# NUStatBioinfo/DegNorm

Measured on AMD Instinct MI355X. Metric: genes/sec (20k genes x 10 samples, 5 iters), higher is better.
Workload: dtype f64

## Files before the change

### degnorm_amd/csrc/dn_api.hip

```cpp
#include "dn_kernels.hpp"
#include "dn_host.hpp"
#include "dn_outer.hpp"
#include "../../include/degnorm_amd.h"

#include <dlfcn.h>
#include <rccl/rccl.h>

#include <algorithm>
#include <atomic>
#include <cmath>
#include <cstdio>
#include <cstdlib>
#include <cstring>
#include <memory>
#include <numeric>
#include <string>
#include <thread>
#include <vector>

#ifndef DN_P_MAX_TEMPLATED
#define DN_P_MAX_TEMPLATED 64
#endif
#define DN_P_2_16(X)  X(2) X(3) X(4) X(5) X(6) X(7) X(8) X(9) X(10) X(11) X(12) X(13) X(14) X(15) X(16)
#define DN_P_17_24(X) X(17) X(18) X(19) X(20) X(21) X(22) X(23) X(24)
// ... 299 lines not shown
#ifndef DN_BUILD_STAMP
#define DN_BUILD_STAMP "unknown build"
#endif
const char *dn_version(void) { return "degnorm_amd 0.2.0 (gfx950) [" DN_BUILD_STAMP "]"; }
const char *dn_last_error(void) { return dn::last_error(); }
const char *dn_reads_last_error(void) { return dn::last_error(); }
const char *dn_assemble_last_error(void) { return dn::last_error(); }
const char *dn_gtf_last_error(void) { return dn::last_error(); }

int dn_device_count(void)
{
    int n = 0;
    if (hipGetDeviceCount(&n) != hipSuccess) return 0;
    return n;
}

int dn_p_supported(int p) { return p <= dn::P_MAX && dn::kernel_set_for(p) != nullptr; }
int dn_p_max(void) { return dn::P_WIDE_MAX; }

static int create_streams(dn_handle h)
{
    int prio_least = 0, prio_greatest = 0;
    DN_TRY(hipDeviceGetStreamPriorityRange(&prio_least, &prio_greatest));
    const int prio[dn_handle_s::NCLS] = {prio_greatest, (prio_least + prio_greatest) / 2, prio_least};
    for (int c = 0; c < dn_handle_s::NCLS; c++) {
        DN_TRY(h->stream[c].create(hipStreamCreateWithPriority, hipStreamNonBlocking, prio[c]));
        DN_TRY(h->ev_start[c].create(hipEventCreate));
        DN_TRY(h->ev_end[c].create(hipEventCreate));
        DN_TRY(h->ev_mid[c].create(hipEventCreateWithFlags, hipEventDisableTiming));
    }
    DN_TRY(h->ev_ready.create(hipEventCreateWithFlags, hipEventDisableTiming));
    DN_TRY(h->ev_i0.create(hipEventCreate));
    DN_TRY(h->ev_i1.create(hipEventCreate));
    return DN_OK;
}

int dn_create(int device, dn_handle *out)
{
    if (!out) return fail(DN_E_INVALID, "dn_create: out is null");
    *out = nullptr;
    int ndev = 0;
    if (hipGetDeviceCount(&ndev) != hipSuccess || ndev <= 0) return fail(DN_E_NO_DEVICE, "no HIP device visible");
    if (device < 0 || device >= ndev) return fail(DN_E_INVALID, "dn_create: device index out of range");
    DN_TRY(hipSetDevice(device));
    hipDeviceProp_t prop;
    DN_TRY(hipGetDeviceProperties(&prop, device));
    dn_handle h = std::make_unique<dn_handle_s>().release();
    h->device = device;
    h->n_cus = prop.multiProcessorCount;
    const int rc = create_streams(h);
    if (rc != DN_OK) {
        const std::string msg = g_err;
        (void) dn_destroy(h);
        return fail(rc, msg);
    }
    *out = h;
    return DN_OK;
}

int dn_destroy(dn_handle h)
{
    if (!h) return DN_OK;
    (void) hipSetDevice(h->device);
    wait_streams(h);
    (void) dn_comm_destroy(h);
    delete h;
    return DN_OK;
}

static int64_t lds_tier_cols(const dn::KernelSet *ks, int per_cu, int32_t p)
{
    const int64_t lds_per_block = (160 * 1024) / per_cu - (int64_t) ks->static_lds_bytes - 256;
    const int64_t ps = p + (p & 1);
    return lds_per_block > 0 ? lds_per_block / std::max(1, ks->units) / (8 * ps) : 0;
}

static int size_class(dn_handle h, dn_handle_s::GeneClass &C, int32_t cols)
{
    const int32_t p = h->p;
    int per_cu = C.ks->blocks_per_cu(0);
    if (per_cu < 1) per_cu = 1;
    const int units = std::max(1, C.ks->units);
    int slots = (int) std::min<int64_t>(((int64_t) C.n + units - 1) / units * units, (int64_t) per_cu * h->n_cus * units);
    const int32_t S = (cols + 63) & ~63;
    const int64_t slot_bytes = (int64_t) S * ((int64_t) p * 2 * sizeof(float) + (int64_t) (p + (p & 1)) * sizeof(double) + 3 * sizeof(double)) +
                               (int64_t) C.ks->slot_extra_bytes;
    {
        size_t free_b = 0, total_b = 0;
        DN_TRY(hipMemGetInfo(&free_b, &total_b));
        const int64_t budget = (int64_t) ((free_b + (C.d_ws ? (size_t) C.slot_bytes * (size_t) std::max(C.slots, 1) : 0)) / 3);
        if (slot_bytes > budget) return fail(DN_E_INVALID, "a gene is too long for the device scratch (" + std::to_string(S) + " columns)");
        slots = (int) std::max<int64_t>(units, std::min<int64_t>(slots, budget / slot_bytes / units * units));
    }
    dn::DeviceBuffer<char> ws;
    DN_TRY(ws.alloc((size_t) slot_bytes * (size_t) std::max(slots, 1)));
    C.d_ws = std::move(ws);
    C.slots = slots; C.S = S; C.slot_bytes = slot_bytes;
    const int64_t lcols = std::min<int64_t>(lds_tier_cols(C.ks, per_cu, p), C.S) & ~(int64_t) 1;
    C.lds_cols = (int32_t) lcols;
    C.dyn_lds = (size_t) units * (size_t) lcols * 8 * (size_t) (p + (p & 1));
    return DN_OK;
}

struct CoverageSource {
    const float *packed = nullptr;
    const void *const *genes = nullptr;
    int32_t is_f32 = 0, n_threads = 1;
    std::atomic<int64_t> *bad = nullptr;
};

static void pack_genes(dn_handle h, const CoverageSource &src, int64_t g0, int64_t g1, float *stage)
{
    const int32_t p = h->p;
    const int64_t base = h->goff[g0];
    std::atomic<int64_t> next(g0);
    auto work = [&]() {
        int64_t local_bad = 0;
        for (;;) {
            const int64_t a = next.fetch_add(16);
            if (a >= g1) break;
            const int64_t b = std::min(g1, a + 16);
            for (int64_t g = a; g < b; g++) {
                const int64_t cnt = (int64_t) p * h->glen[g];
                float *dst = stage + (h->goff[g] - base);
                if (src.is_f32) std::memcpy(dst, src.genes[g], sizeof(float) * (size_t) cnt);
                else {
                    const double *s = (const double *) src.genes[g];
                    for (int64_t k = 0; k < cnt; k++) { const float f = (float) s[k]; dst[k] = f; local_bad += ((double) f != s[k]); }
                }
            }
        }
        if (src.bad) *src.bad += local_bad;
    };
    const int nt = (int) std::max<int64_t>(1, std::min<int64_t>(src.n_threads, (g1 - g0 + 15) / 16));
    std::vector<std::thread> th;
    for (int t = 1; t < nt; t++) th.emplace_back(work);
    work();
    for (auto &t : th) t.join();
}

static int upload_ragged_chunks(dn_handle h, const CoverageSource &src, dn::PinnedBuffer<float> (&stage)[2], dn::Event (&done)[2])
{
    const int64_t n = h->n;
    int64_t chunk = (int64_t) 32 << 20;
    if (const char *env = getenv("DN_UPLOAD_CHUNK_FLOATS")) chunk = std::max<int64_t>(1, atoll(env));
    for (int64_t g = 0; g < n; g++) chunk = std::max(chunk, (int64_t) h->p * h->glen[g]);
    chunk = std::min(chunk, std::max<int64_t>(h->total, 1));
    for (int b = 0; b < 2; b++) {
        if (stage[b].alloc(sizeof(float) * (size_t) chunk) != hipSuccess ||
            done[b].create(hipEventCreateWithFlags, hipEventDisableTiming) != hipSuccess) return fail(DN_E_HIP, "upload: pinned staging buffer");
    }
    int64_t g0 = 0;
    for (int k = 0; g0 < n; k++) {
        int64_t g1 = g0, fl = 0;
        while (g1 < n && fl + (int64_t) h->p * h->glen[g1] <= chunk) { fl += (int64_t) h->p * h->glen[g1]; g1++; }
        const int b = k & 1;
        if (k >= 2 && hipEventSynchronize(done[b]) != hipSuccess) return fail(DN_E_HIP, "upload: event");
        pack_genes(h, src, g0, g1, stage[b]);
        if (hipMemcpyAsync(h->data.d_cov + h->goff[g0], stage[b], sizeof(float) * (size_t) fl, hipMemcpyHostToDevice, h->stream[0]) != hipSuccess ||
            hipEventRecord(done[b], h->stream[0]) != hipSuccess) return fail(DN_E_HIP, "upload: copy");
        g0 = g1;
    }
    if (hipStreamSynchronize(h->stream[0]) != hipSuccess) return fail(DN_E_HIP, "upload: synchronize");
    return DN_OK;
}

static void class_lengths(const dn::KernelSet *ks, int32_t p, int32_t &split_len, int32_t &tiny_len, const dn::KernelSet *&pair)
{
    {
        const char *env = getenv("DN_SPLIT_LEN");
        const dn::KernelSet *narrow = (ks->p != 0) ? dn::kernel_set_narrow(p) : nullptr;
        split_len = 0;
        if (env) split_len = atoi(env);
        else if (narrow) {
            const int64_t lds_cols_n = lds_tier_cols(narrow, std::max(1, narrow->blocks_per_cu(0)), p);
            const int64_t reg_cols_n = narrow->reg_tier_cols;
            split_len = (int32_t) (reg_cols_n > 0 ? (int64_t) (1.775 * (double) (reg_cols_n + lds_cols_n)) : (int64_t) (2.1 * (double) lds_cols_n));
        }
        if (!narrow) split_len = 0;
        if (!env && p >= 25) split_len = 0;
        pair = (ks->p != 0 && split_len > 0) ? dn::kernel_set_pair(p) : nullptr;
// ... 1072 lines not shown
```

### degnorm_amd/csrc/dn_kernels.hpp

```cpp
#pragma once
#include <hip/hip_runtime.h>
#include <stddef.h>
#include <stdint.h>
#include <type_traits>
#include "dn_reduce.hpp"
#include "dn_dpp_ops.hpp"

#ifdef DN_MARKS
#define DN_MARK(name) asm volatile("; DN_MARK " name)
#else
#define DN_MARK(name)
#endif

namespace dn {

constexpr int TRACE_LEN = 48;
constexpr int MAX_BINS = 64;
constexpr int P_MAX = 64;
constexpr int P_WIDE_MAX = 256;

enum { EXIT_LOW_COV = 0, EXIT_ZERO_SAMPLE = 1, EXIT_MEDIAN = 2, EXIT_NO_LOOP = 3,
       EXIT_REFINED = 4, EXIT_REFINE_FALLBACK = 5, EXIT_NOT_FOUND_FALLBACK = 6 };
enum { LOOP_NATURAL = 0, LOOP_PERFECT = 1, LOOP_VALUE_ERROR = 2, LOOP_ZERO_ROWSUM = 3, LOOP_MIN_BINS = 4,
       LOOP_NOT_ENTERED = 5 };
enum { ST_OK = 0, ST_ARPACK = -1, ST_EMPTY_MIN = -2, ST_VALUE_ERROR = -3,
       ST_NO_CONVERGENCE = -4 };
constexpr int EIG_MAX_STEPS_DEFAULT = 4000;
enum { EM_INPUT = 0,
       EM_EXPAND = 1,
       EM_REFINED = 2,
       EM_CLAMPED = 3,
       EM_RAW = 4 };

template <typename CovT>
struct IterFields {
    const CovT    *cov;
    const int64_t *goff;
    const int32_t *glen;
    const int32_t *order;
    int32_t       *counter;
    const int64_t *ds_start;
    const CovT    *rowmax;
    const int32_t *x16;
    char          *ws;
    double        *rho;
    int32_t       *flags;
    int32_t       *trace;
    double        *kfin;
    int32_t       *emode;
    double        *svec;
    const int64_t *svoff;
    int64_t        slot_bytes;
    int32_t        n_genes;
    int32_t        S;
    int32_t        lds_cols;
    int32_t        T, bins, min_hc, rate, skip, want_est;
    int32_t        p;
    int32_t        max_steps;
    int32_t        handdown_cols;
    int32_t       *hand_int;
    double        *hand_dbl;
    int32_t       *park_queue;
    int32_t       *park_count;
    const int32_t *resume_queue;
    const int32_t *resume_count;
};
constexpr int HAND_MAX_BINS = 32;
constexpr int HAND_INTS = 16 + HAND_MAX_BINS;

struct IterArgs : IterFields<float> { double scale[P_MAX], inv_scale[P_MAX]; };

struct IterArgsF64 : IterFields<double> { double scale[P_MAX], inv_scale[P_MAX]; };

struct WideIterArgs : IterFields<float> { const double *scale, *inv_scale; };

struct InitArgs {
    const float   *cov;
    const int64_t *goff;
    const int32_t *glen;
    const int32_t *order;
    int32_t       *counter;
    double        *est_sums;
    double        *cov_sums;
    int32_t       *status;
    int32_t        n_genes;
    int32_t        p;
    int32_t        max_steps;
    char          *ws;
    int64_t        slot_bytes;
    int32_t        S;
    const int32_t *x16;
    int32_t        force_fp64;
};

template <typename CovT>
struct EstFields {
    const CovT    *cov;
    const int64_t *goff;
    const int32_t *glen;
    const double  *kfin;
    const int32_t *emode;
    const double  *svec;
    const int64_t *svoff;
    double        *out;
    const int64_t *ooff;
    int32_t        n_genes;
    int32_t        p;
};
struct EstArgs : EstFields<float> { double scale[P_MAX]; };
struct EstArgsF64 : EstFields<double> { double scale[P_MAX]; };
struct WideEstArgs : EstFields<float> { const double *scale; };

#pragma clang diagnostic push
#pragma clang diagnostic ignored "-Winvalid-offsetof"
template <typename A> constexpr bool iter_layout_kept()
{
    return sizeof(A) == 1256 && offsetof(A, slot_bytes) == 128 && offsetof(A, p) == 172 && offsetof(A, hand_int) == 184 &&
           offsetof(A, scale) == 232 && offsetof(A, inv_scale) == 744;
}
template <typename A> constexpr bool est_layout_kept() { return sizeof(A) == 592 && offsetof(A, p) == 76 && offsetof(A, scale) == 80; }
static_assert(iter_layout_kept<IterArgs>() && iter_layout_kept<IterArgsF64>(), "IterArgs / IterArgsF64: layout moved");
static_assert(est_layout_kept<EstArgs>() && est_layout_kept<EstArgsF64>(), "EstArgs / EstArgsF64: layout moved");
#pragma clang diagnostic pop

struct NmfArgsF64 {
    const double  *x;
    const int64_t *xoff;
    const int32_t *ncol;
    const int64_t *eoff;
    const int32_t *order;
    int32_t       *counter;
    double        *K;
    double        *E;
    double        *est;
    int32_t       *status;
    char          *ws;
    int64_t        slot_bytes;
    int32_t        n, p, T, ratio, max_steps;
};

#ifndef DN_MG_MIN_P
#define DN_MG_MIN_P 25
#endif

template <int P, int NT>
struct Smem {
    static constexpr int W = NT / 64;
    static constexpr int MG_TR = (P + 15) / 16;
    static constexpr int MG_STR = 16 * MG_TR;
// ... 768 lines not shown
#define g_sm g_sm_u[DN_UNIT]
#define g_gs g_gs_u[DN_UNIT]
typedef const float __attribute__((address_space(1))) *gF_cptr;
typedef double __attribute__((address_space(1))) *gdouble_ptr;

template <int P>
__device__ __forceinline__ void col_update(const double (&f)[P], double (&a)[P], const double (&u)[P], const double (&ur)[P], double c)
{
    double s0 = 0.0, s1 = 0.0;
#pragma unroll
    for (int i = 0; i + 1 < P; i += 2) { s0 = fma(u[i], a[i], s0); s1 = fma(u[i + 1], a[i + 1], s1); }
    if (P & 1) s0 = fma(u[P - 1], a[P - 1], s0);
    const double s = s0 + s1;
#pragma unroll
    for (int i = 0; i < P; i++) {
        const double res = fma(ur[i], s, -f[i]);
        a[i] = fmax(fma(-c, res, a[i]), f[i]);
    }
}

template <int P>
__device__ __forceinline__ void col_update_lds(const float (&x)[P], const double *invp, double (&a)[P], const double *uv, double c)
{
    double s0 = 0.0, s1 = 0.0;
#pragma unroll
    for (int i = 0; i + 1 < P; i += 2) {
        const double2 u2 = *reinterpret_cast<const double2 *>(uv + i);
        s0 = fma(u2.x, a[i], s0); s1 = fma(u2.y, a[i + 1], s1);
    }
    if (P & 1) s0 = fma(uv[P - 1], a[P - 1], s0);
    const double s = s0 + s1;
#pragma unroll
    for (int i = 0; i < P; i++) {
        const double fi = (double) x[i] * invp[i];
        const double res = fma(uv[i], s, -fi);
        a[i] = fmax(fma(-c, res, a[i]), fi);
    }
}

template <int P>
__device__ __forceinline__ void col_final(const double (&f)[P], const double (&a)[P], const double (&u)[P], bool first,
                                          double (&acc)[2 * P + 1], double &s_out, double &r_out)
{
    double s = 0.0;
#pragma unroll
    for (int i = 0; i < P; i++) s = fma(u[i], a[i], s);
    acc[0] += s;
    double rmax = 0.0;
#pragma unroll
    for (int i = 0; i < P; i++) {
        const double ke = u[i] * s;
        acc[1 + i] += ke < f[i] ? f[i] : ke;
        acc[1 + P + i] += f[i];
        double d = ke - f[i];
        if (!first) d = d < 0.0 ? 0.0 : d;
        const double r = d * rcp_newton(f[i] + 1.0);
        const double r2 = r * r;
        rmax = r2 > rmax ? r2 : rmax;
    }
    s_out = s; r_out = rmax;
}

template <int PS>
__device__ __forceinline__ void lds_col_read(const double *col, double (&a)[PS])
{
#pragma unroll
    for (int i = 0; i < PS; i += 2) { const double2 v = *reinterpret_cast<const double2 *>(col + i); a[i] = v.x; a[i + 1] = v.y; }
}
template <int PS>
__device__ __forceinline__ void lds_col_write(double *col, const double (&a)[PS])
{
#pragma unroll
    for (int i = 0; i < PS; i += 2) *reinterpret_cast<double2 *>(col + i) = make_double2(a[i], a[i + 1]);
}

typedef float dn_f4 __attribute__((ext_vector_type(4)));
typedef float dn_f2 __attribute__((ext_vector_type(2)));
typedef dn_f4 dn_f4u __attribute__((aligned(4)));
typedef dn_f2 dn_f2u __attribute__((aligned(4)));
typedef const dn_f4u __attribute__((address_space(1))) *gF4_cptr;
typedef const dn_f2u __attribute__((address_space(1))) *gF2_cptr;

template <int P>
__device__ __forceinline__ void load_x(gF_cptr Fb, int k, float (&x)[P])
{
    gF_cptr col = Fb + (size_t) k * P;
#pragma unroll
    for (int i = 0; i + 4 <= P; i += 4) {
        const dn_f4 v = *(gF4_cptr) (col + i);
        x[i] = v.x; x[i + 1] = v.y; x[i + 2] = v.z; x[i + 3] = v.w;
    }
    if constexpr ((P & 3) >= 2) {
        const dn_f2 v = *(gF2_cptr) (col + (P & ~3));
        x[P & ~3] = v.x; x[(P & ~3) + 1] = v.y;
    }
    if constexpr (P & 1) x[P - 1] = col[P - 1];
}

template <int P>
__device__ __forceinline__ void load_f(gF_cptr Fb, int k, const double (&inv)[P], double (&f)[P])
{
    float x[P];
    load_x<P>(Fb, k, x);
#pragma unroll
    for (int i = 0; i < P; i++) f[i] = (double) x[i] * inv[i];
}

template <int P, bool RAW>
__device__ __forceinline__ void pass_counts(const float (&x)[P], const double (&inv)[P], double (&f)[P])
{
#pragma unroll
    for (int i = 0; i < P; i++) f[i] = RAW ? (double) x[i] : (double) x[i] * inv[i];
}

typedef double dn_d2 __attribute__((ext_vector_type(2)));
typedef dn_d2 __attribute__((address_space(1))) *gd2_ptr;
template <int P> constexpr int spill_mid() { return (P + (P & 1)) / 4; }
template <int P>
__device__ __forceinline__ gd2_ptr spill_col(gdouble_ptr Lg, int k)
{
    constexpr int PS = P + (P & 1);
    gd2_ptr col = (gd2_ptr) (Lg + ((size_t) (k >> 6) * (64 * PS) + (size_t) (k & 63) * 2)) + spill_mid<P>() * 64;
    asm volatile("" : "+v"(col));
    return col;
}
template <int P>
__device__ __forceinline__ void spill_col_read(gd2_ptr col, double (&a)[P])
{
#pragma unroll
    for (int q = 0; q < (P + 1) / 2; q++) {
        const dn_d2 v = col[(q - spill_mid<P>()) * 64];
        a[2 * q] = v.x;
        if (2 * q + 1 < P) a[2 * q + 1] = v.y;
    }
}
template <int P>
__device__ __forceinline__ void spill_col_write(gd2_ptr col, const double (&a)[P])
{
#pragma unroll
    for (int q = 0; q < (P + 1) / 2; q++) col[(q - spill_mid<P>()) * 64] = dn_d2{a[2 * q], 2 * q + 1 < P ? a[2 * q + 1 < P ? 2 * q + 1 : 2 * q] : 0.0};
}

template <int P, int NT>
__device__ __forceinline__ int mg_core(gF_cptr Fb, gdouble_ptr Lg, double *lam, int n, int nL, int T,
                                       double (&u)[P], double &theta, int &steps, int maxs, bool &noconv)
{
    constexpr int W = NT / 64;
    constexpr int NG = P * (P + 1) / 2;
    constexpr int PS = P + (P & 1);
    constexpr int TR = Smem<P, NT>::MG_TR, STR = Smem<P, NT>::MG_STR;
    constexpr int NTILE = TR * (TR + 1) / 2;
    Smem<P, NT> &sm = g_sm;
    const int tid = DN_TIDX, lane = lane_id(), w = wave_id();
    const int nLe = (n < nL) ? n : nL;
    double *stage = &sm.stage[w * 16 * STR];
    double *uv = &sm.eigv[w * 128], *vv = uv + 64;
    const double *invp = g_gs.inv;
    for (int e = lane; e < 16 * STR; e += 64) stage[e] = 0.0;
    uv[lane] = lane < P ? 1.0 / sqrt((double) P) : 0.0;
    vv[lane] = 0.0;
    wave_fence();
    const int oi = lane & 15, okq = lane >> 4;
    dn_double4 acc[NTILE];

    auto feed = [&](const double (&a)[PS], bool valid) {
#pragma unroll
        for (int cq = 0; cq < 4; cq++) {
            if ((lane >> 4) == cq) {
                double *dst = stage + (lane & 15) * STR;
#pragma unroll
                for (int i = 0; i < PS; i += 2) *reinterpret_cast<double2 *>(dst + i) = make_double2(valid ? a[i] : 0.0, valid ? a[i + 1] : 0.0);
            }
            wave_fence();
#pragma unroll
            for (int g = 0; g < 4; g++) {
                double x[TR];
#pragma unroll
                for (int tr = 0; tr < TR; tr++) x[tr] = stage[(4 * g + okq) * STR + 16 * tr + oi];
                int tix = 0;
// ... 192 lines not shown
template <int IDX> __device__ __forceinline__ void agpr_put(double v)
{
    agpr_put1<IDX>(__double2loint(v));
    agpr_put1<IDX + 1>(__double2hiint(v));
}

template <int P, int BASE> __device__ __forceinline__ void rt_read(double (&a)[P])
{
    static_for<0, P>([&](auto ic) { constexpr int I = decltype(ic)::value; a[I] = agpr_get<BASE + 2 * I>(); });
}
template <int P, int BASE> __device__ __forceinline__ void rt_write(const double (&a)[P])
{
    static_for<0, P>([&](auto ic) { constexpr int I = decltype(ic)::value; agpr_put<BASE + 2 * I>(a[I]); });
}
template <int P, int BASE> __device__ __forceinline__ void rt_read_counts(double (&xd)[P])
{
    static_for<0, (P + 1) / 2>([&](auto jc) {
        constexpr int J = decltype(jc)::value;
        const unsigned w = (unsigned) agpr_get1<BASE + J>();
        xd[2 * J] = (double) (w & 0xffffu);
        if constexpr (2 * J + 1 < P) xd[2 * J + 1] = (double) (w >> 16);
    });
}
template <int P, int BASE> __device__ __forceinline__ void rt_write_counts(const float (&x)[P])
{
    static_for<0, (P + 1) / 2>([&](auto jc) {
        constexpr int J = decltype(jc)::value;
        unsigned w = (unsigned) x[2 * J];
        if constexpr (2 * J + 1 < P) w |= ((unsigned) x[2 * J + 1]) << 16;
        agpr_put1<BASE + J>((int) w);
    });
}
template <int P, bool X16> constexpr int rt_col_regs() { return 2 * P + (X16 ? (P + 1) / 2 : 0); }
template <int P, bool X16> constexpr int rt_cols()
{
    return (P >= DN_RT_MIN_P && P <= DN_RT_MAX_P) ? (256 / rt_col_regs<P, X16>() < DN_RT_MAX_COLS ? 256 / rt_col_regs<P, X16>() : DN_RT_MAX_COLS) : 0;
}
template <int P> constexpr int rt_regs_used()
{
    return rt_cols<P, true>() * rt_col_regs<P, true>() > rt_cols<P, false>() * rt_col_regs<P, false>()
               ? rt_cols<P, true>() * rt_col_regs<P, true>() : rt_cols<P, false>() * rt_col_regs<P, false>();
}
constexpr int RT_BATCH = 48;
#define DN_RT_SAVE_IDX(r) ((size_t) (r) * NT + DN_TIDX)
template <int N, int NT> __device__ __forceinline__ void rt_save(int *save, int need)
{
    static_for<0, (N + RT_BATCH - 1) / RT_BATCH>([&](auto bc) {
        constexpr int B = decltype(bc)::value * RT_BATCH;
        constexpr int CNT = (N - B) < RT_BATCH ? (N - B) : RT_BATCH;
        if (B < need) {
            int v[CNT];
            static_for<0, CNT>([&](auto ic) { constexpr int I = decltype(ic)::value; v[I] = agpr_get1<B + I>(); });
#pragma unroll
            for (int i = 0; i < CNT; i++) save[DN_RT_SAVE_IDX(B + i)] = v[i];
            asm volatile("" ::: "memory");
        }
    });
}
template <int N, int NT> __device__ __forceinline__ void rt_restore(const int *save, int need)
{
    static_for<0, (N + RT_BATCH - 1) / RT_BATCH>([&](auto bc) {
        constexpr int B = decltype(bc)::value * RT_BATCH;
        constexpr int CNT = (N - B) < RT_BATCH ? (N - B) : RT_BATCH;
        if (B < need) {
            int v[CNT];
#pragma unroll
            for (int i = 0; i < CNT; i++) v[i] = save[DN_RT_SAVE_IDX(B + i)];
            static_for<0, CNT>([&](auto ic) { constexpr int I = decltype(ic)::value; agpr_put1<B + I>(v[I]); });
            asm volatile("" ::: "memory");
        }
    });
}
template <int R, int RT, typename F>
__device__ __forceinline__ void partial_rounds(int nr, F &&column)
{
    if constexpr (R < RT) {
        if (R == 0 || R < nr) {
            column(std::integral_constant<int, R>{});
            __builtin_amdgcn_sched_barrier(0);
            partial_rounds<R + 1, RT>(nr, column);
        }
    }
}
template <int P, int NT> constexpr size_t rt_save_bytes() { return (size_t) rt_regs_used<P>() * 4 * NT; }

template <int P, int NT, bool X16, bool FULL = false, bool ONCHIP = false, bool SAFE = false>
__device__ __forceinline__ void nmf_body(const float *Fb_, double *Lg_, double *rs_, double *sv_,
                                         int n, int S, int nL, int T, int first_i)
{
    Smem<P, NT> &sm = g_sm;
    double *lam = g_lam + (DN_UNITS > 1 ? (size_t) DN_UNIT * (size_t) nL * (P + (P & 1)) : 0);
    gF_cptr Fb = (gF_cptr) uniform_ptr(Fb_);
    gdouble_ptr Lg = (gdouble_ptr) uniform_ptr(Lg_);
    gdouble_ptr rs = (gdouble_ptr) uniform_ptr(rs_);
    gdouble_ptr sv = (gdouble_ptr) uniform_ptr(sv_);
    n = __builtin_amdgcn_readfirstlane(n);
    S = __builtin_amdgcn_readfirstlane(S);
    nL = __builtin_amdgcn_readfirstlane(nL);
    T = __builtin_amdgcn_readfirstlane(T);
    const bool first = __builtin_amdgcn_readfirstlane(first_i) != 0;
    double inv[P], u[P], theta = 0.0;
    int steps = 0;
    const int maxs = __builtin_amdgcn_readfirstlane(g_gs.max_steps);
    bool noconv = false;
#pragma unroll
    for (int i = 0; i < P; i++) inv[i] = uniform(g_gs.inv[i]);
    long long stamp[4] = {0, 0, 0, 0};
#ifdef DN_STAMP
#define DN_T0() const long long t0_ = __builtin_amdgcn_s_memtime()
#define DN_T1(slot) stamp[slot] += __builtin_amdgcn_s_memtime() - t0_
#else
#define DN_T0()
#define DN_T1(slot) (void) stamp
#endif
    constexpr int NG = P * (P + 1) / 2;
    constexpr int CH_MAX = P <= 15 ? 120 : 90;
    constexpr int SW = (NG + CH_MAX - 1) / CH_MAX;
    constexpr int CH = (NG + SW - 1) / SW;
    constexpr int PS = P + (P & 1);
    const int tid = DN_TIDX;
    constexpr int RT = DN_REG_TIER ? rt_cols<P, X16>() : 0;
    constexpr int CS = rt_col_regs<P, X16>();
    constexpr int NR = RT * NT;
    constexpr bool RAW = raw_units<P>();
    double ud[P], ur[P];
    const int nLe = (n < NR + nL) ? n : NR + nL;
    const int kS0 = NR + nL;
    if constexpr (P >= DN_MG_MIN_P) {
        const int st = mg_core<P, NT>(Fb, Lg, lam, n, nL, T, u, theta, steps, maxs, noconv);
        if (st != ST_OK) { if (tid == 0) g_gs.status = st; dn_sync(); return; }
    } else {
    gram_t G[CH];

#ifdef DN_STAMP
    const long long t_cold0 = __builtin_amdgcn_s_memtime();
#endif
#pragma unroll
    for (int i = 0; i < CH; i++) G[i] = 0.0;
    {
        float xq[P];
        if (tid < n) load_x<P>(Fb, tid, xq);
#pragma clang loop unroll(disable)
        for (int k = tid; k < n; k += NT) {
            double f[P];
#pragma unroll
            for (int i = 0; i < P; i++) f[i] = (double) xq[i] * inv[i];
            load_x<P>(Fb, k + NT < n ? k + NT : k, xq);
            gram_add_range<P, 0, CH>(G, f);
        }
    }
    block_sum_lds<CH, P, NT, gram_t>(G, sm);
    static_for<1, SW>([&](auto qc) {
        constexpr int Q = decltype(qc)::value;
        constexpr int NQ = (NG - Q * CH) < CH ? (NG - Q * CH) : CH;
        gram_t Gq[NQ];
#pragma unroll
        for (int i = 0; i < NQ; i++) Gq[i] = 0.0;
#pragma clang loop unroll(disable)
        for (int k = tid; k < n; k += NT) {
            double f[P];
            load_f<P>(Fb, k, inv, f);
            gram_add_range<P, Q * CH, NQ>(Gq, f);
        }
        block_sum_lds<NQ, P, NT, gram_t, false, Q * CH>(Gq, g_sm);
    });
    {
        double tr = 0.0;
#pragma unroll
        for (int i = 0; i < P; i++) tr += sm.tot[i * (i + 1) / 2 + i];
        if (!(tr > 0.0)) { if (tid == 0) g_gs.status = ST_ARPACK; dn_sync(); return; }
    }
    Solver<P> solver;
    {
        double tr = 0.0;
#pragma unroll
        for (int i = 0; i < P; i++) tr += sm.tot[i * (i + 1) / 2 + i];
        solver.cold(tr, u);
    }
    {
        const int r = SAFE ? solve_by_blocks<P>(solver, sm.tot, Smem<P, NT>::ZSLOT, u, theta, maxs)
                           : solver.run(sm.tot, Smem<P, NT>::ZSLOT, u, theta, T == 0, maxs, true);
        steps += r; noconv = noconv || r > maxs;
    }
    const double c = 1.0 / sqrt((double) T);
    auto pass_u = [&]() {
        if constexpr (RAW) {
            const int k = Solver<P>::row_of_lane() < P ? Solver<P>::row_of_lane() : P - 1;
            const double vt = solver.iterate_of_row() * g_gs.inv[k], vh = solver.iterate_of_row() * g_gs.scl[k];
#pragma unroll
            for (int i = 0; i < P; i++) { ud[i] = Solver<P>::bcast_component(vt, i); ur[i] = Solver<P>::bcast_component(vh, i); }
        } else {
#pragma unroll
            for (int i = 0; i < P; i++) { u[i] = uniform(u[i]); ud[i] = u[i]; ur[i] = u[i]; }
        }
    };
    pass_u();

    constexpr bool PART = RT > 0 && X16 && !FULL;
    const int nr = (n + NT - 1) / NT;
    static_for<0, RT>([&](auto rc) {
        constexpr int R = decltype(rc)::value;
        const int k = tid + R * NT;
        if constexpr (PART) {
            if (R < nr) {
                float xf[P];
                double f[P];
#pragma unroll
                for (int i = 0; i < P; i++) xf[i] = 0.0f;
                if (k < n) load_x<P>(Fb, k, xf);
                pass_counts<P, RAW>(xf, inv, f);
                rt_write<P, CS * R>(f);
                rt_write_counts<P, CS * R + 2 * P>(xf);
            }
        } else if (k < n) {
            float xf[P];
            double f[P];
            load_x<P>(Fb, k, xf);
            pass_counts<P, RAW>(xf, inv, f);
            rt_write<P, CS * R>(f);
            if constexpr (X16) rt_write_counts<P, CS * R + 2 * P>(xf);
        }
    });
    for (int k = NR + tid; k < nLe; k += NT) {
        double f[P], a[PS];
        { float xf[P]; load_x<P>(Fb, k, xf); pass_counts<P, RAW>(xf, inv, f); }
#pragma unroll
        for (int i = 0; i < PS; i++) a[i] = i < P ? f[i] : 0.0;
        lds_col_write<PS>(lam + (size_t) (k - NR) * PS, a);
    }
    if constexpr (!ONCHIP) {
        for (int k = kS0 + tid; k < n; k += NT) {
            double f[P];
            { float xf[P]; load_x<P>(Fb, k, xf); pass_counts<P, RAW>(xf, inv, f); }
            spill_col_write<P>(spill_col<P>(Lg, k), f);
        }
    }
#ifdef DN_STAMP
    stamp[3] += __builtin_amdgcn_s_memtime() - t_cold0;
#endif
    constexpr bool G0 = FULL && ONCHIP && SW == 1;
    constexpr bool SQ = Solver<P>::SQUARE && SW == 1 && !SAFE;
#pragma clang loop unroll(disable)
    for (int t = 0; t < T; t++) {
        DN_MARK("iter_begin");
        auto gram_zero = [&]() {
#pragma unroll
            for (int i = 0; i < CH; i++) G[i] = 0.0;
        };
        if constexpr (!G0 && !PART) gram_zero();
        DN_MARK("zeroed");
        { DN_T0();
        const int dir = (t & 1) ? -1 : 1;

        auto reg_tier = [&](auto start) {
            if constexpr (RT > 0 && X16) {
                auto column = [&](auto rc) {
                    constexpr int R = decltype(rc)::value;
                    double f[P], a[P];
                    rt_read_counts<P, CS * R + 2 * P>(f);
                    if constexpr (!RAW) {
#pragma unroll
                        for (int i = 0; i < P; i++) f[i] *= inv[i];
                    }
                    rt_read<P, CS * R>(a);
                    col_update<P>(f, a, ud, ur, c);
                    if constexpr (decltype(start)::value && R == 0) gram_set_range<P, 0, CH>(G, a); else gram_add_range<P, 0, CH>(G, a);
                    rt_write<P, CS * R>(a);
                };
                if constexpr (FULL) {
                    static_for<0, RT>([&](auto rc) { column(rc); __builtin_amdgcn_sched_barrier(0); });
                } else {
                    partial_rounds<0, RT>(nr, column);
                }
            } else if constexpr (RT > 0) {
                float xq[P];
                if (tid < n) load_x<P>(Fb, tid, xq);
                static_for<0, RT>([&](auto rc) {
                    constexpr int R = decltype(rc)::value;
                    const int k = tid + R * NT;
                    if (k < n) {
                        double f[P], a[P];
                        pass_counts<P, RAW>(xq, inv, f);
                        if constexpr (R + 1 < RT) load_x<P>(Fb, k + NT < n ? k + NT : k, xq);
                        rt_read<P, CS * R>(a);
                        col_update<P>(f, a, ud, ur, c);
                        gram_add_range<P, 0, CH>(G, a);
                        rt_write<P, CS * R>(a);
                    }
                });
            }
        };
        auto lds_tier = [&]() {
            const int first = NR + tid;
            const int cnt = first < nLe ? (nLe - first + NT - 1) / NT : 0;
            const int step = dir * NT;
            int k = dir > 0 ? first : first + (cnt - 1) * NT;
            float xq[P];
            if (cnt > 0) load_x<P>(Fb, k, xq);
#pragma clang loop unroll(disable)
            for (int j = 0; j < cnt; j++, k += step) {
                double f[P], a[PS];
                lds_col_read<PS>(lam + (size_t) (k - NR) * PS, a);
                pass_counts<P, RAW>(xq, inv, f);
                load_x<P>(Fb, j + 1 < cnt ? k + step : k, xq);
                double aa[P];
#pragma unroll
                for (int i = 0; i < P; i++) aa[i] = a[i];
                col_update<P>(f, aa, ud, ur, c);
                gram_add_range<P, 0, CH>(G, aa);
#pragma unroll
                for (int i = 0; i < P; i++) a[i] = aa[i];
                lds_col_write<PS>(lam + (size_t) (k - NR) * PS, a);
            }
        };
        auto spill_tier = [&]() {
            if constexpr (ONCHIP) return;
            int tq = tid;
            asm volatile("" : "+v"(tq));
            const int first = kS0 + tq;
            if (first >= n) return;
            const int step = dir * NT;
            const int last = first + (n - 1 - first) / NT * NT;
            int k = dir > 0 ? first : last;
            const int kend = dir > 0 ? last : first;
            float xn[P];
            double an[P];
            load_x<P>(Fb, k, xn);
            spill_col_read<P>(spill_col<P>(Lg, k), an);
            bool more;
#pragma clang loop unroll(disable)
            do {
                double f[P], a[P];
                pass_counts<P, RAW>(xn, inv, f);
#pragma unroll
                for (int i = 0; i < P; i++) a[i] = an[i];
                const int kn = dir > 0 ? min(k + step, kend) : max(k + step, kend);
                load_x<P>(Fb, kn, xn);
                spill_col_read<P>(spill_col<P>(Lg, kn), an);
                col_update<P>(f, a, ud, ur, c);
                gram_add_range<P, 0, CH>(G, a);
                spill_col_write<P>(spill_col<P>(Lg, k), a);
                more = k != kend;
                k += step;
            } while (more);
        };
#if defined(DN_STAMP) && defined(DN_EXP_TIER)
#define DN_TIER(id, call) do { if (DN_EXP_TIER == id) { const long long tt_ = __builtin_amdgcn_s_memtime(); call; stamp[0] += __builtin_amdgcn_s_memtime() - tt_; } else { call; } } while (0)
#else
#define DN_TIER(id, call) call
#endif
        if constexpr (PART) {
            const bool mem = n > NR;
            if (dir > 0) { DN_MARK("reg_tier"); DN_TIER(1, reg_tier(std::true_type{})); if (mem) { DN_MARK("lds_tier"); DN_TIER(2, lds_tier()); DN_MARK("spill_tier"); DN_TIER(3, spill_tier()); } }
            else { gram_zero(); if (mem) { DN_MARK("spill_tier_b"); DN_TIER(3, spill_tier()); DN_MARK("lds_tier_b"); DN_TIER(2, lds_tier()); } DN_MARK("reg_tier_b"); DN_TIER(1, reg_tier(std::false_type{})); }
        }
        else if constexpr (G0) { DN_MARK("reg_tier"); DN_TIER(1, reg_tier(std::true_type{})); DN_MARK("lds_tier"); DN_TIER(2, lds_tier()); }
        else if (dir > 0) { DN_MARK("reg_tier"); DN_TIER(1, reg_tier(std::false_type{})); DN_MARK("lds_tier"); DN_TIER(2, lds_tier()); DN_MARK("spill_tier"); DN_TIER(3, spill_tier()); }
        else { DN_MARK("spill_tier_b"); DN_TIER(3, spill_tier()); DN_MARK("lds_tier_b"); DN_TIER(2, lds_tier()); DN_MARK("reg_tier_b"); DN_TIER(1, reg_tier(std::false_type{})); }
        DN_MARK("pass_end");
#if !(defined(DN_STAMP) && defined(DN_EXP_TIER))
        DN_T1(0);
#endif
        }
        { DN_T0(); block_sum_lds<CH, P, NT, gram_t, Solver<P>::SHIFTED, 0, RAW, SQ>(G, sm, solver.shift(), solver.scale(), t & 1); DN_T1(1); }
        DN_MARK("reduced");
        static_for<1, SW>([&](auto qc) {
            constexpr int Q = decltype(qc)::value;
            constexpr int NQ = (NG - Q * CH) < CH ? (NG - Q * CH) : CH;
            gram_t Gq[NQ];
#pragma unroll
            for (int i = 0; i < NQ; i++) Gq[i] = 0.0;
            static_assert(SW == 1 || RT == 0, "the later sweeps do not read the register tier");
#pragma clang loop unroll(disable)
            for (int k = NR + tid; k < nLe; k += NT) {
                double a[PS], aa[P];
// ... 681 lines not shown
```

Before: 16020.

## Fully unroll the LDS tier into fixed rounds for p=10 with padded columns

For p=10 the LDS tier now processes a fixed number of rounds (7 × block size) through a compile-time unrolled loop. It uses precomputed byte offsets for the count loads and per-thread LDS column pointers instead of a runtime-strided loop. Host sizing pads the column count to a whole number of rounds plus one, so the tail can be zero-filled and no bounds checks are needed. It fails with an error when LDS cannot hold the rounds. This trades flexibility and some extra scratch for less loop overhead and better scheduling of loads against the column updates.

```diff
diff --git a/degnorm_amd/csrc/dn_api.hip b/degnorm_amd/csrc/dn_api.hip
--- a/degnorm_amd/csrc/dn_api.hip
+++ b/degnorm_amd/csrc/dn_api.hip
@@ -405,7 +405,10 @@
     if (per_cu < 1) per_cu = 1;
     const int units = std::max(1, C.ks->units);
     int slots = (int) std::min<int64_t>(((int64_t) C.n + units - 1) / units * units, (int64_t) per_cu * h->n_cus * units);
-    const int32_t S = (cols + 63) & ~63;
+    const int rounds = C.ks->reg_tier_cols > 0 ? dn::lds_round_count(p) : 0;
+    if (rounds > 0 && lds_tier_cols(C.ks, per_cu, p) < (int64_t) rounds * C.ks->nt)
+        return fail(DN_E_INVALID, "the LDS of a CU does not hold " + std::to_string(rounds) + " rounds of " + std::string(C.ks->baseline_name));
+    const int32_t S = rounds > 0 ? (cols + C.ks->nt - 1) / C.ks->nt * C.ks->nt + C.ks->nt : (cols + 63) & ~63;
     const int64_t slot_bytes = (int64_t) S * ((int64_t) p * 2 * sizeof(float) + (int64_t) (p + (p & 1)) * sizeof(double) + 3 * sizeof(double)) +
                                (int64_t) C.ks->slot_extra_bytes;
     {
@@ -419,7 +422,7 @@
     DN_TRY(ws.alloc((size_t) slot_bytes * (size_t) std::max(slots, 1)));
     C.d_ws = std::move(ws);
     C.slots = slots; C.S = S; C.slot_bytes = slot_bytes;
-    const int64_t lcols = std::min<int64_t>(lds_tier_cols(C.ks, per_cu, p), C.S) & ~(int64_t) 1;
+    const int64_t lcols = rounds > 0 ? (int64_t) rounds * C.ks->nt : std::min<int64_t>(lds_tier_cols(C.ks, per_cu, p), C.S) & ~(int64_t) 1;
     C.lds_cols = (int32_t) lcols;
     C.dyn_lds = (size_t) units * (size_t) lcols * 8 * (size_t) (p + (p & 1));
     return DN_OK;
diff --git a/degnorm_amd/csrc/dn_kernels.hpp b/degnorm_amd/csrc/dn_kernels.hpp
--- a/degnorm_amd/csrc/dn_kernels.hpp
+++ b/degnorm_amd/csrc/dn_kernels.hpp
@@ -65,6 +65,7 @@
     const int32_t *resume_queue;
     const int32_t *resume_count;
 };
+constexpr int lds_round_count(int p) { return p == 10 ? 7 : 0; }
 constexpr int HAND_MAX_BINS = 32;
 constexpr int HAND_INTS = 16 + HAND_MAX_BINS;
 
@@ -999,9 +1000,8 @@
 typedef const dn_f2u __attribute__((address_space(1))) *gF2_cptr;
 
 template <int P>
-__device__ __forceinline__ void load_x(gF_cptr Fb, int k, float (&x)[P])
-{
-    gF_cptr col = Fb + (size_t) k * P;
+__device__ __forceinline__ void load_x_col(gF_cptr col, float (&x)[P])
+{
 #pragma unroll
     for (int i = 0; i + 4 <= P; i += 4) {
         const dn_f4 v = *(gF4_cptr) (col + i);
@@ -1012,6 +1012,20 @@
         x[P & ~3] = v.x; x[(P & ~3) + 1] = v.y;
     }
     if constexpr (P & 1) x[P - 1] = col[P - 1];
+}
+template <int P>
+__device__ __forceinline__ void load_x(gF_cptr Fb, int k, float (&x)[P]) { load_x_col<P>(Fb + (size_t) k * P, x); }
+template <int P>
+__device__ __forceinline__ void load_x_off(gF_cptr Fb, unsigned off, float (&x)[P])
+{
+    load_x_col<P>((gF_cptr) ((const char __attribute__((address_space(1))) *) Fb + off), x);
+}
+template <int P>
+__device__ __forceinline__ void zero_x(gF_cptr Fb, int k)
+{
+    float __attribute__((address_space(1))) *col = const_cast<float __attribute__((address_space(1))) *>(Fb) + (size_t) k * P;
+#pragma unroll
+    for (int i = 0; i < P; i++) col[i] = 0.0f;
 }
 
 template <int P>
@@ -1370,6 +1384,18 @@
         }
     }
 }
+template <int J, int LC, typename F>
+__device__ __forceinline__ void lds_rounds(int nrl, int &r, int step, F &&column)
+{
+    if constexpr (J < LC) {
+        if (J < nrl) {
+            column(r, std::integral_constant<bool, (J + 1 < LC)>{});
+            r += step;
+            __builtin_amdgcn_sched_barrier(0);
+            lds_rounds<J + 1, LC>(nrl, r, step, column);
+        }
+    }
+}
 template <int P, int NT> constexpr size_t rt_save_bytes() { return (size_t) rt_regs_used<P>() * 4 * NT; }
 
 template <int P, int NT, bool X16, bool FULL = false, bool ONCHIP = false, bool SAFE = false>
@@ -1509,9 +1535,22 @@
             if constexpr (X16) rt_write_counts<P, CS * R + 2 * P>(xf);
         }
     });
-    for (int k = NR + tid; k < nLe; k += NT) {
+    constexpr int LC = (RT > 0 && X16 && FULL) ? lds_round_count(P) : 0;
+    constexpr bool LR = LC > 0;
+    static_assert(LC <= 8, "the unrolled LDS tier is meant for a few rounds");
+    const int nrl = (LR && ONCHIP) ? (n - NR + NT - 1) / NT : 0;
+    const int nLp = (LR && ONCHIP) ? NR + nrl * NT : nLe;
+    for (int k = NR + tid; k < nLp; k += NT) {
         double f[P], a[PS];
-        { float xf[P]; load_x<P>(Fb, k, xf); pass_counts<P, RAW>(xf, inv, f); }
+        {
+            float xf[P];
+            if constexpr (LR && ONCHIP) {
+#pragma unroll
+                for (int i = 0; i < P; i++) xf[i] = 0.0f;
+                if (k < n) load_x<P>(Fb, k, xf); else zero_x<P>(Fb, k);
+            } else load_x<P>(Fb, k, xf);
+            pass_counts<P, RAW>(xf, inv, f);
+        }
 #pragma unroll
         for (int i = 0; i < PS; i++) a[i] = i < P ? f[i] : 0.0;
         lds_col_write<PS>(lam + (size_t) (k - NR) * PS, a);
@@ -1579,6 +1618,46 @@
             }
         };
         auto lds_tier = [&]() {
+            if constexpr (LR) {
+                int tq;
+                asm volatile("v_mov_b32 %0, %1" : "=v"(tq) : "v"(tid));
+                double *const ll = lam + (size_t) tq * PS;
+                const unsigned x0 = (unsigned) (NR + tq) * (unsigned) (P * sizeof(float));
+                constexpr unsigned XR = NT * P * sizeof(float);
+                float xq[P];
+                auto column = [&](double *col, auto more, unsigned xnext) {
+                    double f[P], a[PS];
+                    lds_col_read<PS>(col, a);
+                    pass_counts<P, RAW>(xq, inv, f);
+                    if constexpr (decltype(more)::value) load_x_off<P>(Fb, xnext, xq);
+                    double aa[P];
+#pragma unroll
+                    for (int i = 0; i < P; i++) aa[i] = a[i];
+                    col_update<P>(f, aa, ud, ur, c);
+                    gram_add_range<P, 0, CH>(G, aa);
+#pragma unroll
+                    for (int i = 0; i < P; i++) a[i] = aa[i];
+                    lds_col_write<PS>(col, a);
+                };
+                if constexpr (!ONCHIP) {
+                    load_x_off<P>(Fb, x0 + (dir > 0 ? 0 : LC - 1) * XR, xq);
+                    static_for<0, LC>([&](auto jc) {
+                        constexpr int J = decltype(jc)::value;
+                        if (dir > 0) column(ll + J * NT * PS, std::integral_constant<bool, (J + 1 < LC)>{}, x0 + (J + 1) * XR);
+                        else column(ll + (LC - 1 - J) * NT * PS, std::integral_constant<bool, (J + 1 < LC)>{}, x0 + (LC - 2 - J) * XR);
+                        __builtin_amdgcn_sched_barrier(0);
+                    });
+                } else {
+                    int nq;
+                    asm volatile("s_mov_b32 %0, %1" : "=s"(nq) : "s"(nrl));
+                    int r = dir > 0 ? 0 : (nq > 0 ? nq - 1 : 0);
+                    load_x_off<P>(Fb, x0 + (unsigned) r * XR, xq);
+                    lds_rounds<0, LC>(nq, r, dir, [&](int rr, auto more) {
+                        column(ll + rr * (NT * PS), more, x0 + (unsigned) (rr + dir) * XR);
+                    });
+                }
+                return;
+            }
             const int first = NR + tid;
             const int cnt = first < nLe ? (nLe - first + NT - 1) / NT : 0;
             const int step = dir * NT;
```

Result: no change. 16070, median of 6 (+0.3%).
